# YOUNESELBOUKNIFY/CrossModal-IMU-Video-OOD-HAR

Measured on AMD Instinct MI355X. Metric: clips/sec fwd+bwd, 16x224^2 video + 200x6 IMU, batch 32, 1/2/4/8 GPU, higher is better.
Workload: dtype bf16; 1 GPU; CrossModalModel pretrain step: VideoMAE-B 16x224^2 + IMU 6x200 PatchTST, SigLIP loss, clip 1.0, AdamW; global_batch=32, per_gpu_batch=32, parallelism=dp1

## Files before the change

crossmodal-imu-video-ood-har_amd/cmhar/_lib.py:

```python
from __future__ import annotations

import ctypes as C
import os

import torch

_HERE = os.path.dirname(os.path.abspath(__file__))
LIB_PATH = os.environ.get('CMHAR_LIB', os.path.join(_HERE, 'libcmhar.so'))

F32, BF16, F16 = 0, 1, 2
ACT_NONE, ACT_GELU, ACT_RELU, ACT_DGELU, ACT_DRELU, ACT_GELU_SAVEGRAD, ACT_MULAUX = 0, 1, 2, 3, 4, 5, 6

vp, i32, i64, f32, u64 = C.c_void_p, C.c_int, C.c_long, C.c_float, C.c_ulonglong


class Epilogue(C.Structure):
    _fields_ = [('bias', vp), ('residual', vp), ('ldr', i64), ('aux_in', vp), ('lda', i64), ('aux_out', vp),
                ('ldo', i64), ('rowadd', vp), ('rowadd_mod', i32), ('rowadd_ld', i32), ('act', i32),
                ('alpha', f32), ('beta', f32), ('pdrop', f32), ('pad_', i32), ('seed', u64), ('rowsum', vp),
                ('rowsum_beta', f32), ('colscale_lo', i32), ('colscale_hi', i32), ('colscale', f32)]


class IMULayer(C.Structure):
    _fields_ = ([(n, vp) for n in ('w_qkv', 'b_qkv', 'w_out', 'b_out', 'ln1_g', 'ln1_b', 'w_ff1', 'b_ff1', 'w_ff2',
# ... 9 lines not shown
IMU_MAX_LAYERS = 8

_SIGS = {
    'cmhar_version': (i32, []),
    'cmhar_gemm_bf16': (i32, [i32, i32, i32, i32, i32, vp, i64, vp, i64, vp, i64, C.POINTER(Epilogue), i32, vp, vp]),
    'cmhar_gemm_bf16_phased': (i32, [i32, i32, i32, i32, i32, vp, i64, vp, i64, vp, i64, C.POINTER(Epilogue), i32, vp,
                                     vp, i32]),
    'cmhar_gemm_f16': (i32, [i32, i32, i32, i32, i32, vp, i64, vp, i64, vp, i64, C.POINTER(Epilogue), i32, vp, vp]),
    'cmhar_gemm_bf16_ws': (i64, [i32, i32, i32]),
    'cmhar_gemm_bf16_plan': (i32, [i32, i32, i32, i32, i32, i32, i32]),
    'cmhar_gemm_bf16_plan2': (i32, [i32, i32, i32, i32, i32, i32, i32, i32]),
    'cmhar_gemm_generic': (i32, [i32, i32, i32, i32, i32, i32, vp, i64, i64, i64, vp, i64, i64, i64, vp, i64, i64,
                                 C.POINTER(Epilogue), vp]),
    'cmhar_gemm_generic_splitk': (i32, [i32, i32, i32, i32, i32, i32, vp, i64, i64, vp, i64, i64, vp, i64,
                                        C.POINTER(Epilogue), vp, vp]),
    'cmhar_attention_fwd': (i32, [i32, i32, i32, i32, i32, i32, vp, i64, vp, i64, vp, i64, vp, i64, vp, f32, f32, u64,
                                  vp]),
    'cmhar_attention_fwd_opt': (i32, [i32]),
    'cmhar_attention_bwd': (i32, [i32, i32, i32, i32, i32, i32, vp, i64, vp, i64, vp, i64, vp, i64, vp, i64, vp, vp,
                                  vp, i64, vp, i64, vp, i64, f32, f32, u64, vp]),
    'cmhar_attention_bwd_prescaled': (i32, [i32, i32, i32, i32, vp, i64, vp, i64, vp, i64, vp, i64, vp, i64, vp, vp,
                                            vp, i64, vp, i64, vp, i64, f32, vp]),
    'cmhar_layernorm_fwd': (i32, [i32, i32, i32, vp, i64, vp, i64, f32, u64, vp, i64, vp, i64, vp, vp, vp, vp, f32,
                                  vp]),
    'cmhar_layernorm_bwd_ws': (i64, [i32, i32]),
    'cmhar_layernorm_bwd': (i32, [i32, i32, i32, vp, i64, vp, i64, vp, vp, vp, vp, i64, vp, i64, vp, i64, f32, u64,
                                  vp, vp, f32, vp, vp]),
    'cmhar_colsum_ws': (i64, [i32, i32]),
    'cmhar_colsum': (i32, [i32, i32, i32, vp, i64, vp, f32, f32, vp, i64, vp]),
    'cmhar_batchnorm_fwd': (i32, [i32, i32, vp, vp, vp, vp, vp, vp, vp, vp, i32, f32, f32, i32, vp, vp]),
    'cmhar_batchnorm_bwd': (i32, [i32, i32, vp, vp, vp, vp, vp, vp, vp, vp, vp, i32, i32, f32, vp]),
    'cmhar_l2normalize_fwd': (i32, [i32, i32, vp, vp, vp, f32, vp]),
    'cmhar_l2normalize_bwd': (i32, [i32, i32, vp, vp, vp, vp, f32, vp]),
    'cmhar_siglip_ws': (i64, [i32, i32]),
    'cmhar_siglip_loss': (i32, [i32, i32, i32, vp, vp, vp, vp, vp, vp, i32, i32, vp, i32, i32, vp, vp, vp, vp]),
    'cmhar_tubelet_im2col': (i32, [i32, i32, i32, i32, i32, i32, i32, i32, vp, vp, vp]),
    'cmhar_imu_embed_fwd': (i32, [i32, i32, i32, i32, i32, i32, i32, i32, vp, C.POINTER(vp), C.POINTER(vp), vp, vp,
                                  vp, vp]),
    'cmhar_imu_embed_bwd': (i32, [i32, i32, i32, i32, i32, i32, i32, i32, i32, vp, vp, vp, vp, C.POINTER(vp),
                                  C.POINTER(vp), vp]),
    'cmhar_imu_encoder_fwd': (i32, [i32, i32, i32, i32, i32, i32, vp, C.POINTER(IMULayer), vp, vp, f32, vp, vp, vp,
                                    f32, f32, u64, vp]),
    'cmhar_imu_encoder_bwd': (i32, [i32, i32, i32, i32, i32, i32, vp, C.POINTER(IMULayer), C.POINTER(IMULayerGrad),
                                    vp, vp, vp, vp, vp, vp, vp, f32, f32, u64, vp]),
    'cmhar_copy2d': (i32, [i32, i32, i32, i32, vp, i64, vp, i64, f32, f32, f32, u64, vp]),
    'cmhar_logits_energy': (i32, [i32, i32, i32, vp, i64, f32, vp, vp, vp, vp]),
    'cmhar_sim_topk_ws': (i64, [i32, i32, i32]),
    'cmhar_sim_topk_splits': (i32, [i32, i32, i32]),
    'cmhar_sim_topk': (i32, [i32, i32, i32, i32, i32, vp, i64, vp, i64, i64, vp, vp, vp, vp]),
    'cmhar_class_moments_ws': (i64, [i32, i32, i32]),
    'cmhar_class_moments': (i32, [i32, i32, i32, i32, vp, i64, vp, vp, vp, vp, vp, vp]),
    'cmhar_class_min_dist': (i32, [i32, i32, i32, i32, vp, i64, vp, i64, vp, i64, vp, vp, vp, i64, vp]),
    'cmhar_cross_entropy_ws': (i64, [i32]),
    'cmhar_resize_ksize': (i32, [i32, i32]),
    'cmhar_video_ingest_ws': (i64, [i32, i32, i32, i32, i32]),
    'cmhar_video_ingest': (i32, [i32, i32, vp, i64, i32, i32, vp, i32, i32, vp, vp, i32, vp, vp, i64, vp]),
    'cmhar_imu_preprocess_ws': (i64, [i64, i32, i32]),
    'cmhar_imu_preprocess': (i32, [i32, i32, vp, vp, i64, vp, i32, i32, i64, vp, vp, i32, vp, vp, vp]),
    'cmhar_cross_entropy': (i32, [i32, i32, vp, i64, i64, vp, i64, f32, f32, f32, i32, vp, vp, vp, vp, vp, vp, i64,
                                  i64, f32, f32, vp, vp, vp]),
    'cmhar_mt_grad_norm': (i32, [vp, vp, i32, vp, vp, f32, i32, vp]),
    'cmhar_mt_adamw': (i32, [vp, vp, i32, f32, f32, f32, f32, f32, f32, f32, vp, vp]),
    'cmhar_mt_adamw_clip': (i32, [vp, vp, i32, f32, f32, f32, f32, f32, f32, f32, vp, i32, vp]),
    'cmhar_mt_cast_bf16': (i32, [vp, vp, i32, vp]),
    'cmhar_conv3d_im2col': (i32, [i32, i32, vp, vp, vp, vp]),
    'cmhar_conv3d_col2im': (i32, [i32, vp, vp, vp, i32, vp]),
# ... 119 lines not shown
```

crossmodal-imu-video-ood-har_amd/cmhar/heads.py:

```python
from __future__ import annotations

import torch
import torch.nn as nn

from . import kernels as K
from ._lib import NoReplicate


def _blocks(seq: nn.Sequential):
    mods = list(seq)
    blocks, i = [], 0
    while i < len(mods) - 1:
        lin, bn, act = mods[i], mods[i + 1], mods[i + 2]
        if not (isinstance(lin, nn.Linear) and isinstance(bn, nn.BatchNorm1d) and isinstance(act, nn.ReLU)):
            raise TypeError('unsupported head structure')
        p, step = 0.0, 3
        if i + 3 < len(mods) and isinstance(mods[i + 3], nn.Dropout):
            p, step = mods[i + 3].p, 4
        blocks.append((lin, bn, p))
        i += step
    if not isinstance(mods[-1], nn.Linear):
        raise TypeError('head must end with a Linear')
    return blocks, mods[-1]

# ... 28 lines not shown
                                    bn_momentum(bn, upd), bn.eps, True,
                                    bn.num_batches_tracked if upd else None)
        pd = p if training else 0.0
        if pd > 0:
            yd = torch.empty_like(y)
            K.copy2d(y, yd, pdrop=pd, seed=seed + bi)
        else:
            yd = y
        if save:
            saved.append((h, z, y, sm, sr, pd, use_batch))
        h = yd
    out = K.linear(h, final.weight, final.bias)
    return out, (saved, h)


def _head_backward(seq, st, dout, seed):
    blocks, final = _blocks(seq)
    saved, hlast = st
    grads = {final.weight: K.linear_wgrad(dout, hlast), final.bias: K.colsum(dout)}
    dh = K.linear_dgrad(dout, final.weight)
    for bi in reversed(range(len(blocks))):
        lin, bn, _ = blocks[bi]
        h, z, y, sm, sr, pd, use_batch = saved[bi]
        if pd > 0:
            K.copy2d(dh, dh, pdrop=pd, seed=seed + bi)
        dz, dgw, dgb = K.batchnorm_bwd(z, y, dh, bn.weight, sm, sr, use_batch, True)
        grads[bn.weight], grads[bn.bias] = dgw, dgb
        grads[lin.weight] = K.linear_wgrad(dz, h)
        grads[lin.bias] = K.colsum(dz)
        dh = K.linear_dgrad(dz, lin.weight)
    return dh, grads


class _HeadFn(torch.autograd.Function):
    @staticmethod
    def forward(ctx, x, seq, training, seed, *params):
        out, st = _head_forward(seq, x, training, seed, save=True)
        ctx.seq, ctx.st, ctx.seed, ctx.params = seq, st, seed, params
        return out

    @staticmethod
    def backward(ctx, dout):
        dx, grads = _head_backward(ctx.seq, ctx.st, dout.contiguous(), ctx.seed)
        ctx.st = None
        return (dx, None, None, None) + tuple(grads.get(p) if p.requires_grad else None for p in ctx.params)


def run_head(seq: nn.Sequential, x: torch.Tensor, training: bool, seeds: _Seeds) -> torch.Tensor:
    if training and x.shape[0] <= 1:
        raise ValueError(f'Expected more than 1 value per channel when training, got input size {tuple(x.shape)}')
    x = x.contiguous().float()
    params = [p for p in seq.parameters()]
    has_drop = any(isinstance(m, nn.Dropout) and m.p > 0 for m in seq)
    seed = seeds.next() if (training and has_drop) else 0
    if torch.is_grad_enabled() and (x.requires_grad or any(p.requires_grad for p in params)):
        return _HeadFn.apply(x, seq, training, seed, *params)
    with torch.no_grad():
        return _head_forward(seq, x, training, seed, save=False)[0]


class ProjectionHead(NoReplicate, nn.Module):

    def __init__(self, in_dim, hidden_dim, out_dim):
        super().__init__()
        self.net = nn.Sequential(
            nn.Linear(in_dim, hidden_dim),
            nn.BatchNorm1d(hidden_dim),
            nn.ReLU(inplace=True),
            nn.Linear(hidden_dim, out_dim),
        )
        self._seeds = _Seeds()

    def forward(self, x):
        return run_head(self.net, x, self.training, self._seeds)


class _L2NormFn(torch.autograd.Function):
    @staticmethod
    def forward(ctx, x, eps):
        y, n = K.l2normalize_fwd(x, eps)
        ctx.save_for_backward(y, n)
        ctx.eps = eps
        return y

    @staticmethod
    def backward(ctx, dy):
        y, n = ctx.saved_tensors
        return K.l2normalize_bwd(y, dy, n, ctx.eps), None


def l2_normalize(x: torch.Tensor, eps: float = 1e-12) -> torch.Tensor:
    x = x.contiguous().float()
    if torch.is_grad_enabled() and x.requires_grad:
        return _L2NormFn.apply(x, eps)
    return K.l2normalize_fwd(x, eps)[0]
```

crossmodal-imu-video-ood-har_amd/cmhar/kernels.py:

```python
from __future__ import annotations

import ctypes as C
import math
import os

import torch

from . import _lib as L
from ._lib import call, ptr

class Tracer:
    def __init__(self):
        self.active = False
        self.only = None
        self.records = []

    def begin(self, name=None):
        if not self.active or (self.only is not None and name not in self.only):
            return None
        ev = torch.cuda.Event(enable_timing=True)
        ev.record()
        return ev

    def end(self, ev0, name, flops, nbytes):
# ... 416 lines not shown
    return y, sm, sr


def batchnorm_bwd(x, y, dy, w, sm, sr, training, relu, beta_acc=0.0, dw=None, db=None):
    B, Cc = x.shape
    dx = torch.empty_like(x)
    if dw is None:
        dw = torch.empty(Cc, dtype=torch.float32, device=x.device)
    if db is None:
        db = torch.empty(Cc, dtype=torch.float32, device=x.device)
    for t, n in ((dw, 'dw'), (db, 'db')):
        if t.dtype != torch.float32 or tuple(t.shape) != (Cc,) or not t.is_contiguous():
            raise ValueError(f'batchnorm_bwd: {n} must be a contiguous fp32 [{Cc}] tensor')
    call('cmhar_batchnorm_bwd', B, Cc, ptr(x), ptr(y), ptr(dy.contiguous()), ptr(w), ptr(sm), ptr(sr), ptr(dx),
         ptr(dw), ptr(db), int(training), int(relu), beta_acc, L.stream(x.device))
    return dx, dw, db


def l2normalize_fwd(x, eps=1e-12):
    M, N = x.shape
    y = torch.empty_like(x)
    nrm = torch.empty(M, dtype=torch.float32, device=x.device)
    call('cmhar_l2normalize_fwd', M, N, ptr(x), ptr(y), ptr(nrm), eps, L.stream(x.device))
    return y, nrm


def l2normalize_bwd(y, dy, nrm, eps=1e-12):
    M, N = y.shape
    dx = torch.empty_like(y)
    call('cmhar_l2normalize_bwd', M, N, ptr(y), ptr(dy.contiguous()), ptr(nrm), ptr(dx), eps, L.stream(y.device))
    return dx


def copy2d(src, dst, alpha=1.0, beta=0.0, pdrop=0.0, seed=0):
    _check_2d(src, 'src')
    _check_2d(dst, 'dst')
    if src.shape != dst.shape:
        raise ValueError('copy2d shape')
    call('cmhar_copy2d', L.dtype_code(src.dtype), L.dtype_code(dst.dtype), src.shape[0], src.shape[1], ptr(src),
         src.stride(0), ptr(dst), dst.stride(0), alpha, beta, pdrop, seed, L.stream(src.device))
    return dst


_REDUCTIONS = {'none': 0, 'mean': 1, 'sum': 2}


def cross_entropy(logits, labels=None, *, ignore_index=-100, label_smoothing=0.0, gamma=0.0, alpha=1.0,
                  reduction='mean', loss=None, row_loss=None, pred=None, correct=None, status=None, dlogits=None,
                  grad_scale=1.0, grad_beta=0.0, g_up=None):
    if logits.dim() != 2 or logits.dtype != torch.float32 or not logits.is_cuda:
        raise ValueError('logits: fp32 device matrix expected')
    N, Cc = logits.shape
    if labels is not None and (labels.dtype != torch.int64 or labels.shape != (N,) or not labels.is_contiguous()):
        raise ValueError(f'labels: contiguous int64 [{N}] expected')
    for t, n in ((row_loss, 'row_loss'), (pred, 'pred')):
        if t is not None and (t.numel() != N or not t.is_contiguous()):
            raise ValueError(f'{n}: [{N}] expected')
    if dlogits is not None and (tuple(dlogits.shape) != (N, Cc) or dlogits.dtype != torch.float32):
        raise ValueError('dlogits shape')
    red = _REDUCTIONS[reduction]
    if dlogits is not None and red == 0 and (g_up is None or g_up.numel() != N):
        raise ValueError("reduction='none' needs per-row upstream gradients")
    ws = workspace(L.lib().cmhar_cross_entropy_ws(N), logits.device)
    call('cmhar_cross_entropy', N, Cc, ptr(logits), logits.stride(0), logits.stride(1), ptr(labels), ignore_index,
         label_smoothing, gamma, alpha, red, ptr(loss), ptr(row_loss), ptr(pred), ptr(correct), ptr(status),
         ptr(dlogits), dlogits.stride(0) if dlogits is not None else 0,
# ... 21 lines not shown
```

crossmodal-imu-video-ood-har_amd/cmhar/models.py:

```python
from __future__ import annotations

import math
import os
import warnings

import torch
import torch.nn as nn

from . import kernels as K
from .heads import ProjectionHead, l2_normalize, run_head, _Seeds
from .imu import IMUEncoder, PatchEmbedding
from .cnn2d import MobileNetV2Features, ResNet18Features, run_cnn2d
from .fusion import _TokenMeanFn
from .r3d import R3D18, run_r3d
from .videomae import VideoMAEBackbone, default_videomae_config, run_backbone

__all__ = ['PatchEmbedding', 'IMUEncoder', 'VideoEncoder', 'ProjectionHead', 'CrossModalModel', 'IMUClassifier']


class _LinearFn(torch.autograd.Function):
    @staticmethod
    def forward(ctx, x, weight, bias):
        ctx.save_for_backward(x, weight)
        ctx.has_bias = bias is not None
        return K.linear(x, weight.detach(), None if bias is None else bias.detach())

    @staticmethod
    def backward(ctx, dy):
        x, w = ctx.saved_tensors
        dy = dy.contiguous()
        dx = K.linear_dgrad(dy, w.detach()) if ctx.needs_input_grad[0] else None
        dw = K.linear_wgrad(dy, x) if ctx.needs_input_grad[1] else None
        db = K.colsum(dy) if ctx.has_bias and ctx.needs_input_grad[2] else None
        return dx, dw, db


def linear_fp32(x, lin: nn.Linear):
    x = x.contiguous().float()
    if torch.is_grad_enabled() and (x.requires_grad or lin.weight.requires_grad):
        return _LinearFn.apply(x, lin.weight, lin.bias)
    return K.linear(x, lin.weight.detach(), None if lin.bias is None else lin.bias.detach())


def _videomae_geometry(config):
    m, d = config.model, config.data
    frames = m.videomae_num_frames or d.video_frames_per_window
    image = m.videomae_image_size or (d.video_resize[0] if isinstance(d.video_resize, (tuple, list)) else d.video_resize)
    return default_videomae_config(image_size=image, patch_size=m.videomae_patch_size, num_frames=frames,
                                   tubelet_size=m.videomae_tubelet_size, hidden_size=m.videomae_hidden_size,
                                   num_hidden_layers=m.videomae_num_layers, num_attention_heads=m.videomae_num_heads,
                                   intermediate_size=m.videomae_intermediate_size,
                                   layer_norm_eps=m.videomae_layer_norm_eps, qkv_bias=m.videomae_qkv_bias,
                                   use_mean_pooling=m.videomae_use_mean_pooling)


class VideoEncoder(nn.Module):

    def __init__(self, config):
        super().__init__()
        self.config = config
        model_cfg = config.model
        vb = model_cfg.video_backbone
        self.is_videomae = False
        dt = getattr(model_cfg, 'compute_dtype', 'bf16')
        if isinstance(vb, str) and ('videomae' in vb.lower() or '/' in vb):
            self.is_videomae = True
            if os.path.isdir(vb) and os.path.exists(os.path.join(vb, 'config.json')):
                self.backbone = VideoMAEBackbone.from_pretrained(vb, compute_dtype=dt)
            else:
                if model_cfg.video_pretrained:
                    allow = bool(getattr(model_cfg, 'allow_random_init', False)) or \
                        os.environ.get('CMHAR_ALLOW_RANDOM_INIT', '') == '1'
                    if not allow:
                        raise OSError(f'VideoMAE checkpoint {vb!r} cannot be loaded (not a local HF directory '
# ... 29 lines not shown

    def forward(self, x):
        if x.dim() != 5:
            raise ValueError(f'expected (B, T, C, H, W) video, got {tuple(x.shape)}')
        if isinstance(self.backbone, (ResNet18Features, MobileNetV2Features)):
            B, T = x.shape[:2]
            feats = linear_fp32(run_cnn2d(self.backbone, x, self.training), self.projection)
            return _TokenMeanFn.apply(feats, B, T)
        if not self.is_videomae:
            return linear_fp32(run_r3d(self.backbone, x, self.training), self.projection)
        feat = run_backbone(self.backbone, x, token0_only=True)
        return linear_fp32(feat, self.projection)


class CrossModalModel(nn.Module):

    def __init__(self, config):
        super().__init__()
        self.config = config
        model_cfg = config.model
        self.imu_encoder = IMUEncoder(config)
        self.video_encoder = VideoEncoder(config)
        self.imu_proj = ProjectionHead(model_cfg.imu_d_model, model_cfg.projection_hidden_dim,
                                       model_cfg.projection_dim)
        self.video_proj = ProjectionHead(model_cfg.video_d_model, model_cfg.projection_hidden_dim,
                                         model_cfg.projection_dim)
        self.temperature = nn.Parameter(torch.ones([]) * math.log(10))
        self.bias = nn.Parameter(torch.ones([]) * -10)
        self.overlap_imu = True
        self._side = {}

    def _imu_branch(self, imu):
        imu_feat, _ = self.imu_encoder(imu)
        return l2_normalize(self.imu_proj(imu_feat))

    def forward(self, imu, video):
        if self.overlap_imu and imu.is_cuda:
            cur = torch.cuda.current_stream(imu.device)
            side = self._side.get(imu.device)
            if side is None:
                side = self._side[imu.device] = torch.cuda.Stream(
                    imu.device, priority=int(os.environ.get('CMHAR_IMU_STREAM_PRIORITY', '0')))
            side.wait_stream(cur)
            with torch.cuda.stream(side):
                imu_out = self._imu_branch(imu)
            video_out = l2_normalize(self.video_proj(self.video_encoder(video)))
            cur.wait_stream(side)
            imu_out.record_stream(cur)
            return imu_out, video_out
        imu_out = self._imu_branch(imu)
        return imu_out, l2_normalize(self.video_proj(self.video_encoder(video)))


class IMUClassifier(nn.Module):

    def __init__(self, imu_encoder, config, freeze_encoder=False):
        super().__init__()
        self.imu_encoder = imu_encoder
        self.config = config
        model_cfg = config.model
        if freeze_encoder:
            for param in self.imu_encoder.parameters():
                param.requires_grad = False
        layers = []
        in_dim = model_cfg.imu_d_model
        for hidden_dim in model_cfg.classifier_hidden_dims:
            layers.extend([nn.Linear(in_dim, hidden_dim), nn.BatchNorm1d(hidden_dim), nn.ReLU(inplace=True),
                           nn.Dropout(model_cfg.classifier_dropout)])
            in_dim = hidden_dim
        layers.append(nn.Linear(in_dim, model_cfg.num_classes))
        self.classifier = nn.Sequential(*layers)
        self._seeds = _Seeds()

    def forward(self, imu):
        with torch.set_grad_enabled(self.training or not self.freeze_encoder):
            imu_feat, _ = self.imu_encoder(imu)
        return run_head(self.classifier, imu_feat, self.training, self._seeds)

    @property
    def freeze_encoder(self):
        return not next(self.imu_encoder.parameters()).requires_grad

    def unfreeze_encoder(self):
        for param in self.imu_encoder.parameters():
# ... 2 lines not shown
```

include/cmhar.h:

```cpp
#ifndef CMHAR_H
#define CMHAR_H
#include <hip/hip_runtime_api.h>

#ifdef __cplusplus
extern "C" {
#endif

typedef struct CmharEpilogue {
  const float* bias;
  const void* residual;
  long ldr;
  const void* aux_in;
  long lda;
  void* aux_out;
  long ldo;
  const float* rowadd;
  int rowadd_mod;
  int rowadd_ld;
  int act;
  float alpha;
  float beta;
  float pdrop;
  int pad_;
  unsigned long long seed;
// ... 30 lines not shown
int cmhar_attention_fwd_opt(int mode);
int cmhar_attention_bwd(int dtype, int B, int H, int Lq, int Lk, int D, const void* Q, long ldq, const void* K,
                        long ldk, const void* V, long ldv, const void* O, long ldo, const void* dO, long lddo,
                        const float* lse, float* delta, void* dQ, long lddq, void* dK, long lddk, void* dV, long lddv,
                        float scale, float pdrop, unsigned long long seed, hipStream_t stream);
int cmhar_attention_bwd_prescaled(int B, int H, int Lq, int Lk, const void* Q, long ldq, const void* K, long ldk,
                                  const void* V, long ldv, const void* O, long ldo, const void* dO, long lddo,
                                  const float* lse, float* delta, void* dQ, long lddq, void* dK, long lddk, void* dV,
                                  long lddv, float scale, hipStream_t stream);

int cmhar_layernorm_fwd(int dtype, int M, int N, const void* a, long lda, const void* b, long ldb, float pdrop,
                        unsigned long long seed, void* h_out, long ldh, void* y, long ldy, const float* gamma,
                        const float* beta, float* mean, float* rstd, float eps, hipStream_t stream);
long cmhar_layernorm_bwd_ws(int M, int N);
int cmhar_layernorm_bwd(int dtype, int M, int N, const void* dy, long lddy, const void* h, long ldh,
                        const float* gamma, const float* mean, const float* rstd, const void* dres, long ldres,
                        void* dh, long lddh, void* db_out, long lddb, float pdrop, unsigned long long seed,
                        float* dgamma, float* dbeta, float beta_acc, float* ws, hipStream_t stream);

long cmhar_colsum_ws(int M, int N);
int cmhar_colsum(int dtype, int M, int N, const void* X, long ldx, float* out, float alpha, float beta, float* ws,
                 long ws_floats, hipStream_t stream);

int cmhar_batchnorm_fwd(int B, int C, const float* x, float* y, const float* w, const float* bias, float* rmean,
                        float* rvar, float* smean, float* srstd, int training, float momentum, float eps, int relu,
                        long long* num_batches_tracked, hipStream_t stream);
int cmhar_batchnorm_bwd(int B, int C, const float* x, const float* y, const float* dy, const float* w,
                        const float* smean, const float* srstd, float* dx, float* dw, float* db, int training,
                        int relu, float beta_acc, hipStream_t stream);

int cmhar_l2normalize_fwd(int M, int N, const float* x, float* y, float* norm, float eps, hipStream_t stream);
int cmhar_l2normalize_bwd(int M, int N, const float* y, const float* dy, const float* norm, float* dx, float eps,
                          hipStream_t stream);

long cmhar_siglip_ws(int Ba, int Bb);
int cmhar_siglip_loss(int Ba, int Bb, int D, const float* a, const float* b, const float* t, const float* bias,
                      float* loss, float* da, int a_off, int a_cnt, float* db, int b_off, int b_cnt, float* gt,
                      float* gbias, float* ws, hipStream_t stream);

int cmhar_tubelet_im2col(int out_dtype, int B, int T, int C, int H, int W, int tub, int P, const float* video,
                         void* out, hipStream_t stream);

int cmhar_imu_embed_fwd(int B, int C, int L, int N, int P, int S, int D, int T, const float* x,
                        const float* const* w, const float* const* bias, const float* cls, const float* pos,
                        float* out, hipStream_t stream);
int cmhar_imu_embed_bwd(int B, int C, int L, int N, int P, int S, int D, int T, int Tpos, const float* x,
                        const float* dout, float* dcls, float* dpos, float* const* dw, float* const* db,
                        hipStream_t stream);

#define CMHAR_IMU_MAX_LAYERS 8
typedef struct CmharIMULayer {
  const float *w_qkv, *b_qkv, *w_out, *b_out, *ln1_g, *ln1_b, *w_ff1, *b_ff1, *w_ff2, *b_ff2, *ln2_g, *ln2_b;
  float eps1, eps2;
  float *qkv, *o, *lse, *s1, *mu1, *rs1, *h1, *fd, *s2, *mu2, *rs2, *h2;
} CmharIMULayer;
int cmhar_imu_encoder_fwd(int B, int T, int D, int H, int FF, int nlayers, const float* x, const CmharIMULayer* layers,
                          const float* norm_g, const float* norm_b, float norm_eps, float* enc, float* norm_mu,
                          float* norm_rs, float scale, float pdrop, unsigned long long seed, hipStream_t stream);
typedef struct CmharIMULayerGrad {
  float *dqkv, *da, *dpre, *df2, *gln1, *gln2;
  float *dw_qkv, *db_qkv, *dw_out, *db_out, *dln1_g, *dln1_b, *dw_ff1, *db_ff1, *dw_ff2, *db_ff2, *dln2_g, *dln2_b;
} CmharIMULayerGrad;
int cmhar_imu_encoder_bwd(int B, int T, int D, int H, int FF, int nlayers, const float* x, const CmharIMULayer* layers,
                          const CmharIMULayerGrad* grads, const float* norm_g, const float* norm_mu,
                          const float* norm_rs, const float* d_enc, float* dnorm_g, float* dnorm_b, float* dx,
                          float scale, float pdrop, unsigned long long seed, hipStream_t stream);
// ... 119 lines not shown
```

Before: 741.8 clips/sec.

## Add fused skinny-batch linear+BatchNorm+ReLU kernels for projection heads

Adds dedicated HIP kernels for small-batch (≤64 rows) fp32 linear layers. The forward kernel fuses bias, BatchNorm (batch or running stats, including running-stat updates) and ReLU into the GEMM. The backward kernel computes dx, dW, db and the BatchNorm or L2-normalize backward in one launch. Projection heads and generic small linears use these kernels, replacing separate linear, batchnorm, colsum and l2normalize launches, to cut launch count and tile waste at batch 32. The cost is a large amount of hand-written MFMA code whose correctness and numerics must match the unfused path.

```diff
diff --git a/crossmodal-imu-video-ood-har_amd/cmhar/_lib.py b/crossmodal-imu-video-ood-har_amd/cmhar/_lib.py
--- a/crossmodal-imu-video-ood-har_amd/cmhar/_lib.py
+++ b/crossmodal-imu-video-ood-har_amd/cmhar/_lib.py
@@ -65,6 +65,9 @@
     'cmhar_batchnorm_bwd': (i32, [i32, i32, vp, vp, vp, vp, vp, vp, vp, vp, vp, i32, i32, f32, vp]),
     'cmhar_l2normalize_fwd': (i32, [i32, i32, vp, vp, vp, f32, vp]),
     'cmhar_l2normalize_bwd': (i32, [i32, i32, vp, vp, vp, vp, f32, vp]),
+    'cmhar_skinny_linear_fwd': (i32, [i32, i32, i32, vp, vp, vp, vp, i32, vp, vp, vp, vp, vp, vp, vp, f32, f32, vp, vp]),
+    'cmhar_skinny_linear_bwd': (i32, [i32, i32, i32, vp, vp, vp, vp, vp, vp, i32, vp, vp, f32, vp, vp, vp, vp, vp, vp,
+                                      i32, vp]),
     'cmhar_siglip_ws': (i64, [i32, i32]),
     'cmhar_siglip_loss': (i32, [i32, i32, i32, vp, vp, vp, vp, vp, vp, i32, i32, vp, i32, i32, vp, vp, vp, vp]),
     'cmhar_tubelet_im2col': (i32, [i32, i32, i32, i32, i32, i32, i32, i32, vp, vp, vp]),
diff --git a/crossmodal-imu-video-ood-har_amd/cmhar/heads.py b/crossmodal-imu-video-ood-har_amd/cmhar/heads.py
--- a/crossmodal-imu-video-ood-har_amd/cmhar/heads.py
+++ b/crossmodal-imu-video-ood-har_amd/cmhar/heads.py
@@ -84,6 +84,64 @@
     return dh, grads
 
 
+def fused_ok(seq, x) -> bool:
+    blocks, final = _blocks(seq)
+    if x.dim() != 2 or any(p > 0 for _, _, p in blocks):
+        return False
+    if any(bn.weight is None or bn.bias is None or not K._f32c(bn.weight) or not K._f32c(bn.bias)
+           for _, bn, _ in blocks):
+        return False
+    lins = [b[0] for b in blocks] + [final]
+    if not K.skinny_ok(x, lins[0].weight, lins[0].bias):
+        return False
+    return all(lin.in_features % 4 == 0 and K._f32c(lin.weight) and lin.weight.data_ptr() % 16 == 0 and
+               (lin.bias is None or K._f32c(lin.bias)) for lin in lins[1:])
+
+
+def _bn_modes(bn, training):
+    upd = training and bn.track_running_stats and bn.running_mean is not None
+    use_batch = training or not bn.track_running_stats
+    return upd, use_batch
+
+
+def _head_forward_fused(seq, x, training, save, norm_eps=None):
+    blocks, final = _blocks(seq)
+    h = x
+    saved = []
+    for lin, bn, _ in blocks:
+        upd, use_batch = _bn_modes(bn, training)
+        stats = upd or not use_batch
+        y, z, sm, sr = K.skinny_linear_fwd(h, lin.weight, lin.bias, bn=dict(
+            weight=bn.weight, bias=bn.bias, rmean=bn.running_mean if stats else None,
+            rvar=bn.running_var if stats else None, batch_stats=use_batch, momentum=bn_momentum(bn, upd), eps=bn.eps,
+            num_batches_tracked=bn.num_batches_tracked if upd else None))
+        if save:
+            saved.append((h, z, y, sm, sr, use_batch))
+        h = y
+    out = K.skinny_linear_fwd(h, final.weight, final.bias)
+    nrm = None
+    if norm_eps is not None:
+        out, nrm = K.l2normalize_fwd(out, norm_eps)
+    return out, (saved, h, out if norm_eps is not None else None, nrm)
+
+
+def _head_backward_fused(seq, st, dout, need_dx, norm_eps=None):
+    blocks, final = _blocks(seq)
+    saved, hlast, yn, nrm = st
+    dh, dw, db = K.skinny_linear_bwd(dout, hlast, final.weight, need_dx=bool(blocks) or need_dx,
+                                     need_db=final.bias is not None,
+                                     l2n=(yn, nrm, norm_eps) if norm_eps is not None else None)
+    grads = {final.weight: dw, final.bias: db}
+    for bi in reversed(range(len(blocks))):
+        lin, bn, _ = blocks[bi]
+        h, z, y, sm, sr, use_batch = saved[bi]
+        dh, dw, db, dg, dbt = K.skinny_linear_bwd(dh, h, lin.weight, need_dx=bi > 0 or need_dx,
+                                                  need_db=lin.bias is not None,
+                                                  bn=(z, y, bn.weight, sm, sr, use_batch))
+        grads[bn.weight], grads[bn.bias], grads[lin.weight], grads[lin.bias] = dg, dbt, dw, db
+    return dh, grads
+
+
 class _HeadFn(torch.autograd.Function):
     @staticmethod
     def forward(ctx, x, seq, training, seed, *params):
@@ -98,11 +156,33 @@
         return (dx, None, None, None) + tuple(grads.get(p) if p.requires_grad else None for p in ctx.params)
 
 
-def run_head(seq: nn.Sequential, x: torch.Tensor, training: bool, seeds: _Seeds) -> torch.Tensor:
+class _FusedHeadFn(torch.autograd.Function):
+
+    @staticmethod
+    def forward(ctx, x, seq, training, norm_eps, *params):
+        out, st = _head_forward_fused(seq, x, training, True, norm_eps)
+        ctx.seq, ctx.st, ctx.norm_eps, ctx.params = seq, st, norm_eps, params
+        return out
+
+    @staticmethod
+    def backward(ctx, dout):
+        dx, grads = _head_backward_fused(ctx.seq, ctx.st, dout.contiguous(), ctx.needs_input_grad[0], ctx.norm_eps)
+        ctx.st = None
+        return (dx, None, None, None) + tuple(grads.get(p) if p.requires_grad else None for p in ctx.params)
+
+
+def run_head(seq: nn.Sequential, x: torch.Tensor, training: bool, seeds: _Seeds, norm_eps=None) -> torch.Tensor:
     if training and x.shape[0] <= 1:
         raise ValueError(f'Expected more than 1 value per channel when training, got input size {tuple(x.shape)}')
     x = x.contiguous().float()
     params = [p for p in seq.parameters()]
+    if fused_ok(seq, x):
+        if torch.is_grad_enabled() and (x.requires_grad or any(p.requires_grad for p in params)):
+            return _FusedHeadFn.apply(x, seq, training, norm_eps, *params)
+        with torch.no_grad():
+            return _head_forward_fused(seq, x, training, False, norm_eps)[0]
+    if norm_eps is not None:
+        return l2_normalize(run_head(seq, x, training, seeds), norm_eps)
     has_drop = any(isinstance(m, nn.Dropout) and m.p > 0 for m in seq)
     seed = seeds.next() if (training and has_drop) else 0
     if torch.is_grad_enabled() and (x.requires_grad or any(p.requires_grad for p in params)):
@@ -126,6 +206,9 @@
     def forward(self, x):
         return run_head(self.net, x, self.training, self._seeds)
 
+    def forward_normalized(self, x, eps: float = 1e-12):
+        return run_head(self.net, x, self.training, self._seeds, norm_eps=eps)
+
 
 class _L2NormFn(torch.autograd.Function):
     @staticmethod
diff --git a/crossmodal-imu-video-ood-har_amd/cmhar/kernels.py b/crossmodal-imu-video-ood-har_amd/cmhar/kernels.py
--- a/crossmodal-imu-video-ood-har_amd/cmhar/kernels.py
+++ b/crossmodal-imu-video-ood-har_amd/cmhar/kernels.py
@@ -472,6 +472,87 @@
     return dx
 
 
+HEADS_FUSED = os.environ.get('CMHAR_HEADS_FUSED', '1') != '0'
+SKINNY_MAX_ROWS = 64
+
+
+def _f32c(t):
+    return t.is_cuda and t.dtype == torch.float32 and t.is_contiguous()
+
+
+def skinny_ok(x, w, bias=None):
+    return (HEADS_FUSED and x.dim() == 2 and w.dim() == 2 and _f32c(x) and _f32c(w) and
+            (bias is None or _f32c(bias)) and 1 <= x.shape[0] <= SKINNY_MAX_ROWS and x.shape[1] == w.shape[1] and
+            x.shape[1] % 4 == 0 and x.data_ptr() % 16 == 0 and w.data_ptr() % 16 == 0)
+
+
+def _check_f32c(shape, **tensors):
+    for n, t in tensors.items():
+        if t is not None and (not _f32c(t) or (shape is not None and tuple(t.shape) != tuple(shape))):
+            raise ValueError(f'{n}: expected a contiguous fp32 device tensor' +
+                             (f' of shape {tuple(shape)}' if shape is not None else '') + f', got {tuple(t.shape)} '
+                             f'{t.dtype}')
+
+
+def skinny_linear_fwd(x, w, bias=None, *, bn=None):
+    B, K = x.shape
+    N = w.shape[0]
+    if not skinny_ok(x, w, bias):
+        raise ValueError(f'skinny_linear_fwd: unsupported operands x {tuple(x.shape)} w {tuple(w.shape)}')
+    _check_f32c((N,), bias=bias)
+    y = torch.empty(B, N, dtype=torch.float32, device=x.device)
+    if bn is None:
+        call('cmhar_skinny_linear_fwd', B, K, N, ptr(x), ptr(w), ptr(bias), ptr(y), 0, None, None, None, None, None,
+             None, None, 0.0, 0.0, None, L.stream(x.device))
+        return y
+    rmean, rvar, nbt = bn.get('rmean'), bn.get('rvar'), bn.get('num_batches_tracked')
+    _check_f32c((N,), bn_weight=bn['weight'], bn_bias=bn['bias'], rmean=rmean, rvar=rvar)
+    if nbt is not None and (nbt.dtype != torch.int64 or nbt.numel() != 1 or not nbt.is_cuda):
+        raise ValueError('num_batches_tracked: expected a device int64 scalar')
+    mode = 1 if bn['batch_stats'] else 2
+    if mode == 2 and (rmean is None or rvar is None):
+        raise ValueError('skinny_linear_fwd: running statistics needed without batch statistics')
+    z = torch.empty_like(y)
+    sm = torch.empty(N, dtype=torch.float32, device=x.device)
+    sr = torch.empty(N, dtype=torch.float32, device=x.device)
+    call('cmhar_skinny_linear_fwd', B, K, N, ptr(x), ptr(w), ptr(bias), ptr(y), mode, ptr(z), ptr(bn['weight']),
+         ptr(bn['bias']), ptr(rmean), ptr(rvar), ptr(sm), ptr(sr), float(bn['momentum']), float(bn['eps']),
+         ptr(nbt) if mode == 1 else None, L.stream(x.device))
+    return y, z, sm, sr
+
+
+def skinny_linear_bwd(dout, x, w, *, need_dx=True, need_db=True, l2n=None, bn=None):
+    B, K = x.shape
+    N = w.shape[0]
+    if not skinny_ok(x, w) or l2n is not None and bn is not None:
+        raise ValueError(f'skinny_linear_bwd: unsupported operands x {tuple(x.shape)} w {tuple(w.shape)}')
+    _check_f32c((B, N), dout=dout)
+    dev = x.device
+    dx = torch.empty(B, K, dtype=torch.float32, device=dev) if need_dx else None
+    dw = torch.empty(N, K, dtype=torch.float32, device=dev)
+    db = torch.empty(N, dtype=torch.float32, device=dev) if need_db else None
+    st = L.stream(dev)
+    if l2n is not None:
+        y, nrm, eps = l2n
+        _check_f32c((B, N), y=y)
+        _check_f32c((B,), norm=nrm)
+        call('cmhar_skinny_linear_bwd', B, K, N, ptr(dout), ptr(x), ptr(w), ptr(dx), ptr(dw), ptr(db), 1, ptr(y),
+             ptr(nrm), float(eps), None, None, None, None, None, None, 0, st)
+        return dx, dw, db
+    if bn is not None:
+        z, y, gw, sm, sr, batch_stats = bn
+        _check_f32c((B, N), z=z, y=y)
+        _check_f32c((N,), bn_weight=gw, smean=sm, srstd=sr)
+        dg = torch.empty(N, dtype=torch.float32, device=dev)
+        dbt = torch.empty(N, dtype=torch.float32, device=dev)
+        call('cmhar_skinny_linear_bwd', B, K, N, ptr(dout), ptr(x), ptr(w), ptr(dx), ptr(dw), ptr(db), 2, ptr(y),
+             None, 0.0, ptr(z), ptr(gw), ptr(sm), ptr(sr), ptr(dg), ptr(dbt), int(batch_stats), st)
+        return dx, dw, db, dg, dbt
+    call('cmhar_skinny_linear_bwd', B, K, N, ptr(dout), ptr(x), ptr(w), ptr(dx), ptr(dw), ptr(db), 0, None, None,
+         0.0, None, None, None, None, None, None, 0, st)
+    return dx, dw, db
+
+
 def copy2d(src, dst, alpha=1.0, beta=0.0, pdrop=0.0, seed=0):
     _check_2d(src, 'src')
     _check_2d(dst, 'dst')
diff --git a/crossmodal-imu-video-ood-har_amd/cmhar/models.py b/crossmodal-imu-video-ood-har_amd/cmhar/models.py
--- a/crossmodal-imu-video-ood-har_amd/cmhar/models.py
+++ b/crossmodal-imu-video-ood-har_amd/cmhar/models.py
@@ -8,7 +8,7 @@
 import torch.nn as nn
 
 from . import kernels as K
-from .heads import ProjectionHead, l2_normalize, run_head, _Seeds
+from .heads import ProjectionHead, run_head, _Seeds
 from .imu import IMUEncoder, PatchEmbedding
 from .cnn2d import MobileNetV2Features, ResNet18Features, run_cnn2d
 from .fusion import _TokenMeanFn
@@ -19,16 +19,24 @@
 
 
 class _LinearFn(torch.autograd.Function):
+
     @staticmethod
     def forward(ctx, x, weight, bias):
         ctx.save_for_backward(x, weight)
         ctx.has_bias = bias is not None
+        ctx.skinny = K.skinny_ok(x, weight, bias)
+        if ctx.skinny:
+            return K.skinny_linear_fwd(x, weight.detach(), None if bias is None else bias.detach())
         return K.linear(x, weight.detach(), None if bias is None else bias.detach())
 
     @staticmethod
     def backward(ctx, dy):
         x, w = ctx.saved_tensors
         dy = dy.contiguous()
+        if ctx.skinny and ctx.needs_input_grad[1]:
+            dx, dw, db = K.skinny_linear_bwd(dy, x, w.detach(), need_dx=ctx.needs_input_grad[0],
+                                             need_db=ctx.has_bias and ctx.needs_input_grad[2])
+            return dx, dw, db
         dx = K.linear_dgrad(dy, w.detach()) if ctx.needs_input_grad[0] else None
         dw = K.linear_wgrad(dy, x) if ctx.needs_input_grad[1] else None
         db = K.colsum(dy) if ctx.has_bias and ctx.needs_input_grad[2] else None
@@ -39,7 +47,8 @@
     x = x.contiguous().float()
     if torch.is_grad_enabled() and (x.requires_grad or lin.weight.requires_grad):
         return _LinearFn.apply(x, lin.weight, lin.bias)
-    return K.linear(x, lin.weight.detach(), None if lin.bias is None else lin.bias.detach())
+    w, b = lin.weight.detach(), None if lin.bias is None else lin.bias.detach()
+    return K.skinny_linear_fwd(x, w, b) if K.skinny_ok(x, w, b) else K.linear(x, w, b)
 
 
 def _videomae_geometry(config):
@@ -135,7 +144,7 @@
 
     def _imu_branch(self, imu):
         imu_feat, _ = self.imu_encoder(imu)
-        return l2_normalize(self.imu_proj(imu_feat))
+        return self.imu_proj.forward_normalized(imu_feat)
 
     def forward(self, imu, video):
         if self.overlap_imu and imu.is_cuda:
@@ -147,12 +156,12 @@
             side.wait_stream(cur)
             with torch.cuda.stream(side):
                 imu_out = self._imu_branch(imu)
-            video_out = l2_normalize(self.video_proj(self.video_encoder(video)))
+            video_out = self.video_proj.forward_normalized(self.video_encoder(video))
             cur.wait_stream(side)
             imu_out.record_stream(cur)
             return imu_out, video_out
         imu_out = self._imu_branch(imu)
-        return imu_out, l2_normalize(self.video_proj(self.video_encoder(video)))
+        return imu_out, self.video_proj.forward_normalized(self.video_encoder(video))
 
 
 class IMUClassifier(nn.Module):
diff --git a/crossmodal-imu-video-ood-har_amd/csrc/heads_fused.hip b/crossmodal-imu-video-ood-har_amd/csrc/heads_fused.hip
--- /dev/null
+++ b/crossmodal-imu-video-ood-har_amd/csrc/heads_fused.hip
@@ -0,0 +1,384 @@
+#include "rowops.h"
+
+namespace {
+
+constexpr int SK_NW = 8, SK_NT = SK_NW * 64;
+constexpr int SK_MAXB = 64;
+constexpr int SK_RLD = 17;
+constexpr int SK_DYF = 12544;
+
+__device__ __forceinline__ floatx4 ld4(const float* p, bool ok) {
+  if (ok) return *(const floatx4*)p;
+  return floatx4{0.f, 0.f, 0.f, 0.f};
+}
+__device__ __forceinline__ float ld1(const float* p, bool ok) { return ok ? *p : 0.f; }
+
+struct SkinnyBN {
+  int mode;
+  float* z;
+  const float* gamma;
+  const float* beta;
+  float* rmean;
+  float* rvar;
+  float* smean;
+  float* srstd;
+  float momentum, eps;
+  long long* nbt;
+};
+
+template <int NBT>
+__global__ __launch_bounds__(SK_NT) void skinny_fwd_kernel(int B, int K, int N, int nc, const float* __restrict__ x,
+                                                           const float* __restrict__ W,
+                                                           const float* __restrict__ bias, float* __restrict__ y,
+                                                           SkinnyBN bn) {
+  __shared__ float red[SK_NW][NBT * 16][SK_RLD];
+  __shared__ float stat[2][16];
+  const int tid = threadIdx.x, lane = tid & 63, w = tid >> 6;
+  const int r = lane & 15, g = lane >> 4;
+  const int n0 = blockIdx.x * nc;
+  const bool nok = r < nc && n0 + r < N;
+  const float* wp = W + (long)(nok ? n0 + r : 0) * K;
+  const float* xp[NBT];
+  bool bok[NBT];
+#pragma unroll
+  for (int bt = 0; bt < NBT; ++bt) {
+    bok[bt] = bt * 16 + r < B;
+    xp[bt] = x + (long)(bok[bt] ? bt * 16 + r : 0) * K;
+  }
+  const int je = tid & 15;
+  const bool jok = je < nc && n0 + je < N;
+  const float bj = ld1(bias + (jok ? n0 + je : 0), jok && bias);
+  const float gj = ld1(bn.gamma + (jok ? n0 + je : 0), jok && bn.mode);
+  const float bej = ld1(bn.beta + (jok ? n0 + je : 0), jok && bn.mode);
+  floatx4 acc[NBT];
+#pragma unroll
+  for (int bt = 0; bt < NBT; ++bt) acc[bt] = floatx4{0.f, 0.f, 0.f, 0.f};
+  constexpr int U = NBT <= 2 ? 3 : 2;
+  for (int kb = w * 32; kb < K; kb += U * SK_NW * 32) {
+    floatx4 wf[U][2], xf[U][NBT][2];
+#pragma unroll
+    for (int u = 0; u < U; ++u) {
+      const int k = kb + u * SK_NW * 32 + 8 * g;
+      const bool k0ok = k < K, k1ok = k + 4 < K;
+      wf[u][0] = ld4(wp + k, nok && k0ok);
+      wf[u][1] = ld4(wp + k + 4, nok && k1ok);
+#pragma unroll
+      for (int bt = 0; bt < NBT; ++bt) {
+        xf[u][bt][0] = ld4(xp[bt] + k, bok[bt] && k0ok);
+        xf[u][bt][1] = ld4(xp[bt] + k + 4, bok[bt] && k1ok);
+      }
+    }
+#pragma unroll
+    for (int u = 0; u < U; ++u)
+#pragma unroll
+      for (int h = 0; h < 2; ++h)
+#pragma unroll
+        for (int e = 0; e < 4; ++e)
+#pragma unroll
+          for (int bt = 0; bt < NBT; ++bt)
+            acc[bt] = __builtin_amdgcn_mfma_f32_16x16x4f32(xf[u][bt][h][e], wf[u][h][e], acc[bt], 0, 0, 0);
+  }
+#pragma unroll
+  for (int bt = 0; bt < NBT; ++bt)
+#pragma unroll
+    for (int rr = 0; rr < 4; ++rr) red[w][bt * 16 + 4 * g + rr][r] = acc[bt][rr];
+  __syncthreads();
+  for (int idx = tid; idx < NBT * 256; idx += SK_NT) {
+    const int b = idx >> 4, j = idx & 15, n = n0 + j;
+    float s = red[0][b][j];
+#pragma unroll
+    for (int ww = 1; ww < SK_NW; ++ww) s += red[ww][b][j];
+    const bool ok = b < B && j < nc && n < N;
+    if (ok && bias) s += bj;
+    red[0][b][j] = s;
+    if (ok) (bn.mode ? bn.z : y)[(long)b * N + n] = s;
+  }
+  if (!bn.mode) return;
+  __syncthreads();
+  if (tid < 16 && tid < nc && n0 + tid < N) {
+    const int c = n0 + tid;
+    float mu, rs;
+    if (bn.mode == 1) {
+      float s = 0.f;
+      for (int b = 0; b < B; ++b) s += red[0][b][tid];
+      mu = s / B;
+      float q = 0.f;
+      for (int b = 0; b < B; ++b) { const float d = red[0][b][tid] - mu; q += d * d; }
+      const float var = q / B;
+      rs = rsqrtf(var + bn.eps);
+      if (bn.rmean) {
+        bn.rmean[c] = (1.f - bn.momentum) * bn.rmean[c] + bn.momentum * mu;
+        bn.rvar[c] = (1.f - bn.momentum) * bn.rvar[c] + bn.momentum * var * B / (B - 1);
+      }
+    } else {
+      mu = bn.rmean[c];
+      rs = rsqrtf(bn.rvar[c] + bn.eps);
+    }
+    bn.smean[c] = mu;
+    bn.srstd[c] = rs;
+    stat[0][tid] = mu;
+    stat[1][tid] = rs;
+  }
+  if (blockIdx.x == 0 && tid == 0 && bn.mode == 1 && bn.nbt) *bn.nbt += 1;
+  __syncthreads();
+  for (int idx = tid; idx < NBT * 256; idx += SK_NT) {
+    const int b = idx >> 4, j = idx & 15, n = n0 + j;
+    if (b < B && j < nc && n < N) {
+      const float v = (red[0][b][j] - stat[0][j]) * stat[1][j] * gj + bej;
+      y[(long)b * N + n] = fmaxf(v, 0.f);
+    }
+  }
+}
+
+struct SkinnyPro {
+  int mode;
+  const float* y;
+  const float* norm;
+  float eps;
+  const float* z;
+  const float* gamma;
+  const float* smean;
+  const float* srstd;
+  float* dgamma;
+  float* dbeta;
+  int training;
+};
+
+template <int NBT>
+__global__ __launch_bounds__(SK_NT) void skinny_bwd_kernel(int B, int K, int N, int nch, const float* __restrict__ dout,
+                                                           const float* __restrict__ x, const float* __restrict__ W,
+                                                           float* __restrict__ dx, float* __restrict__ dW,
+                                                           float* __restrict__ db, SkinnyPro pro) {
+  __shared__ float smem[SK_DYF];
+  __shared__ float rowdot[SK_MAXB], rownorm[SK_MAXB];
+  const int tid = threadIdx.x, lane = tid & 63, w = tid >> 6;
+  const int r = lane & 15, g = lane >> 4;
+  const int k0 = blockIdx.x * 16;
+  const bool kok = k0 + r < K;
+  const int LD = nch + 2;
+  constexpr int B16 = NBT * 16;
+
+  float xr[NBT * 4];
+#pragma unroll
+  for (int s = 0; s < NBT * 4; ++s) {
+    const int b = 4 * s + g;
+    xr[s] = ld1(x + (long)(b < B ? b : 0) * K + (kok ? k0 + r : 0), kok && b < B);
+  }
+  if (pro.mode == 1) {
+    constexpr int RW = (B16 + SK_NW - 1) / SK_NW;
+    float s[RW];
+#pragma unroll
+    for (int i = 0; i < RW; ++i) s[i] = 0.f;
+    for (int c = lane; c < N; c += 256) {
+      float yv[4][RW], dv[4][RW];
+#pragma unroll
+      for (int u = 0; u < 4; ++u)
+#pragma unroll
+        for (int i = 0; i < RW; ++i) {
+          const bool ok = w + SK_NW * i < B && c + 64 * u < N;
+          const long o = ok ? (long)(w + SK_NW * i) * N + c + 64 * u : 0;
+          yv[u][i] = ld1(pro.y + o, ok);
+          dv[u][i] = ld1(dout + o, ok);
+        }
+#pragma unroll
+      for (int u = 0; u < 4; ++u)
+#pragma unroll
+        for (int i = 0; i < RW; ++i) s[i] += yv[u][i] * dv[u][i];
+    }
+#pragma unroll
+    for (int i = 0; i < RW; ++i) {
+      const int bb = w + SK_NW * i;
+      const float t = wave_sum(s[i]);
+      if (lane == 0 && bb < B) { rowdot[bb] = t; rownorm[bb] = pro.norm[bb]; }
+    }
+    __syncthreads();
+  }
+  floatx4 adx[NBT];
+#pragma unroll
+  for (int bt = 0; bt < NBT; ++bt) adx[bt] = floatx4{0.f, 0.f, 0.f, 0.f};
+
+  for (int c0 = 0; c0 < N; c0 += nch) {
+    constexpr int WU = 12;
+    float wf[WU];
+    if (dx) {
+#pragma unroll
+      for (int u = 0; u < WU; ++u) {
+        const int nn = 4 * w + 4 * SK_NW * u, n = c0 + nn + g;
+        const bool ok = kok && n < N && nn < nch;
+        wf[u] = ld1(W + (ok ? (long)n * K + k0 + r : 0), ok);
+      }
+    }
+    if (pro.mode == 2) {
+      constexpr int RB = 32;
+      for (int nn = tid; nn < nch; nn += SK_NT) {
+        const int c = c0 + nn;
+        if (c < N) {
+          const float mu = pro.smean[c], rs = pro.srstd[c], wr = pro.gamma[c] * rs;
+          float gq[RB], xh[RB];
+          auto rows = [&](int b0) {
+#pragma unroll
+            for (int i = 0; i < RB; ++i) {
+              const bool ok = b0 + i < B;
+              const int o = (ok ? b0 + i : 0) * N + c;
+              const float d = dout[o], ya = pro.y[o], zz = pro.z[o];
+              gq[i] = ok && ya > 0.f ? d : 0.f;
+              xh[i] = (zz - mu) * rs;
+            }
+          };
+          float sg = 0.f, sgx = 0.f;
+          for (int b0 = 0; b0 < B; b0 += RB) {
+            rows(b0);
+#pragma unroll
+            for (int i = 0; i < RB; ++i) { sg += gq[i]; sgx += gq[i] * xh[i]; }
+          }
+          if (blockIdx.x == 0) { pro.dgamma[c] = sgx; pro.dbeta[c] = sg; }
+          const float mg = pro.training ? sg / B : 0.f, mgx = pro.training ? sgx / B : 0.f;
+          for (int b0 = 0; b0 < B16; b0 += RB) {
+            if (B > RB) rows(b0);
+#pragma unroll
+            for (int i = 0; i < RB; ++i)
+              if (b0 + i < B16) smem[(b0 + i) * LD + nn] = b0 + i < B ? wr * (gq[i] - mg - xh[i] * mgx) : 0.f;
+          }
+        } else {
+          for (int b = 0; b < B16; ++b) smem[b * LD + nn] = 0.f;
+        }
+      }
+    } else {
+      constexpr int RPT = B16 / 4;
+      const int tc = tid & 127, rg = tid >> 7;
+      for (int nn = tc; nn < nch; nn += 128) {
+        const int c = c0 + nn;
+        float v[RPT], yv[RPT];
+#pragma unroll
+        for (int i = 0; i < RPT; ++i) {
+          const int bb = rg + 4 * i;
+          const bool ok = bb < B && c < N;
+          const int o = ok ? bb * N + c : 0;
+          const float d = dout[o];
+          v[i] = ok ? d : 0.f;
+          yv[i] = pro.mode == 1 ? pro.y[o] : 0.f;
+        }
+#pragma unroll
+        for (int i = 0; i < RPT; ++i) {
+          const int bb = rg + 4 * i;
+          float t = v[i];
+          if (pro.mode == 1 && bb < B) {
+            const float nr = rownorm[bb];
+            t = nr > pro.eps ? (t - yv[i] * rowdot[bb]) / nr : t / pro.eps;
+          }
+          smem[bb * LD + nn] = t;
+        }
+      }
+    }
+    __syncthreads();
+    if (db && blockIdx.x == 0) {
+      for (int nn = tid; nn < nch; nn += SK_NT) {
+        if (c0 + nn < N) {
+          float s = 0.f;
+          for (int b = 0; b < B; ++b) s += smem[b * LD + nn];
+          db[c0 + nn] = s;
+        }
+      }
+    }
+    if (dx) {
+#pragma unroll
+      for (int u = 0; u < WU; ++u) {
+        if (4 * w + 4 * SK_NW * u < nch) {
+#pragma unroll
+          for (int bt = 0; bt < NBT; ++bt)
+            adx[bt] = __builtin_amdgcn_mfma_f32_16x16x4f32(smem[(bt * 16 + r) * LD + 4 * w + 4 * SK_NW * u + g], wf[u],
+                                                           adx[bt], 0, 0, 0);
+        }
+      }
+      for (int nn = 4 * w + 4 * SK_NW * WU; nn < nch; nn += 4 * SK_NW) {
+        const int n = c0 + nn + g;
+        const bool ok = kok && n < N;
+        const float wl = ld1(W + (ok ? (long)n * K + k0 + r : 0), ok);
+#pragma unroll
+        for (int bt = 0; bt < NBT; ++bt)
+          adx[bt] = __builtin_amdgcn_mfma_f32_16x16x4f32(smem[(bt * 16 + r) * LD + nn + g], wl, adx[bt], 0, 0, 0);
+      }
+    }
+    for (int nt = w; nt * 16 < nch && c0 + nt * 16 < N; nt += SK_NW) {
+      floatx4 a = floatx4{0.f, 0.f, 0.f, 0.f};
+#pragma unroll
+      for (int s = 0; s < NBT * 4; ++s)
+        a = __builtin_amdgcn_mfma_f32_16x16x4f32(smem[(4 * s + g) * LD + nt * 16 + r], xr[s], a, 0, 0, 0);
+#pragma unroll
+      for (int rr = 0; rr < 4; ++rr) {
+        const int n = c0 + nt * 16 + 4 * g + rr;
+        if (n < N && kok) dW[(long)n * K + k0 + r] = a[rr];
+      }
+    }
+    __syncthreads();
+  }
+  if (!dx) return;
+  float* red = smem;
+#pragma unroll
+  for (int bt = 0; bt < NBT; ++bt)
+#pragma unroll
+    for (int rr = 0; rr < 4; ++rr) red[(w * B16 + bt * 16 + 4 * g + rr) * SK_RLD + r] = adx[bt][rr];
+  __syncthreads();
+  for (int idx = tid; idx < B16 * 16; idx += SK_NT) {
+    const int b = idx >> 4, j = idx & 15;
+    float s = red[b * SK_RLD + j];
+#pragma unroll
+    for (int ww = 1; ww < SK_NW; ++ww) s += red[(ww * B16 + b) * SK_RLD + j];
+    if (b < B && k0 + j < K) dx[(long)b * K + k0 + j] = s;
+  }
+}
+
+static_assert(SK_NW * SK_MAXB * SK_RLD <= SK_DYF, "dx partial tiles must fit the dy image");
+
+inline bool aligned16(const void* p) { return ((uintptr_t)p & 15) == 0; }
+
+}
+
+extern "C" int cmhar_skinny_linear_fwd(int B, int K, int N, const float* x, const float* W, const float* bias,
+                                       float* y, int bn_mode, float* z, const float* gamma, const float* beta,
+                                       float* rmean, float* rvar, float* smean, float* srstd, float momentum,
+                                       float eps, long long* num_batches_tracked, hipStream_t st) {
+  if (B <= 0 || N <= 0) return 0;
+  if (B > SK_MAXB || K <= 0 || K % 4 || !aligned16(x) || !aligned16(W) || !x || !W || !y) return -1;
+  if (bn_mode < 0 || bn_mode > 2) return -1;
+  if (bn_mode && (!z || !gamma || !beta || !smean || !srstd)) return -1;
+  if (bn_mode == 2 && (!rmean || !rvar)) return -1;
+  if (bn_mode == 1 && (!rmean) != (!rvar)) return -1;
+  SkinnyBN bn{bn_mode, z, gamma, beta, rmean, rvar, smean, srstd, momentum, eps, num_batches_tracked};
+  const int nc = cdiv(N, 16) >= 32 ? 16 : 8;
+  const int grid = cdiv(N, nc);
+  switch (cdiv(B, 16)) {
+    case 1: skinny_fwd_kernel<1><<<grid, SK_NT, 0, st>>>(B, K, N, nc, x, W, bias, y, bn); break;
+    case 2: skinny_fwd_kernel<2><<<grid, SK_NT, 0, st>>>(B, K, N, nc, x, W, bias, y, bn); break;
+    case 3: skinny_fwd_kernel<3><<<grid, SK_NT, 0, st>>>(B, K, N, nc, x, W, bias, y, bn); break;
+    default: skinny_fwd_kernel<4><<<grid, SK_NT, 0, st>>>(B, K, N, nc, x, W, bias, y, bn); break;
+  }
+  CMHAR_CHECK_LAUNCH();
+  return 0;
+}
+
+extern "C" int cmhar_skinny_linear_bwd(int B, int K, int N, const float* dout, const float* x, const float* W,
+                                       float* dx, float* dW, float* db, int pro_mode, const float* py,
+                                       const float* norm, float eps, const float* z, const float* gamma,
+                                       const float* smean, const float* srstd, float* dgamma, float* dbeta,
+                                       int training, hipStream_t st) {
+  if (B <= 0 || N <= 0 || K <= 0) return 0;
+  if (B > SK_MAXB || !dout || !x || !W || !dW) return -1;
+  if (pro_mode < 0 || pro_mode > 2) return -1;
+  if (pro_mode == 1 && (!py || !norm)) return -1;
+  if (pro_mode == 2 && (!py || !z || !gamma || !smean || !srstd || !dgamma || !dbeta)) return -1;
+  SkinnyPro pro{pro_mode, py, norm, eps, z, gamma, smean, srstd, dgamma, dbeta, training};
+  const int nbt = cdiv(B, 16);
+  int nch = ((SK_DYF / (nbt * 16) - 2) / 64) * 64;
+  const int n64 = cdiv(N, 64) * 64;
+  if (nch > n64) nch = n64;
+  const int grid = cdiv(K, 16);
+  switch (nbt) {
+    case 1: skinny_bwd_kernel<1><<<grid, SK_NT, 0, st>>>(B, K, N, nch, dout, x, W, dx, dW, db, pro); break;
+    case 2: skinny_bwd_kernel<2><<<grid, SK_NT, 0, st>>>(B, K, N, nch, dout, x, W, dx, dW, db, pro); break;
+    case 3: skinny_bwd_kernel<3><<<grid, SK_NT, 0, st>>>(B, K, N, nch, dout, x, W, dx, dW, db, pro); break;
+    default: skinny_bwd_kernel<4><<<grid, SK_NT, 0, st>>>(B, K, N, nch, dout, x, W, dx, dW, db, pro); break;
+  }
+  CMHAR_CHECK_LAUNCH();
+  return 0;
+}
diff --git a/include/cmhar.h b/include/cmhar.h
--- a/include/cmhar.h
+++ b/include/cmhar.h
@@ -86,6 +86,15 @@
 int cmhar_l2normalize_fwd(int M, int N, const float* x, float* y, float* norm, float eps, hipStream_t stream);
 int cmhar_l2normalize_bwd(int M, int N, const float* y, const float* dy, const float* norm, float* dx, float eps,
                           hipStream_t stream);
+
+int cmhar_skinny_linear_fwd(int B, int K, int N, const float* x, const float* W, const float* bias, float* y,
+                            int bn_mode, float* z, const float* gamma, const float* beta, float* rmean, float* rvar,
+                            float* smean, float* srstd, float momentum, float eps, long long* num_batches_tracked,
+                            hipStream_t stream);
+int cmhar_skinny_linear_bwd(int B, int K, int N, const float* dout, const float* x, const float* W, float* dx,
+                            float* dW, float* db, int pro_mode, const float* y, const float* norm, float eps,
+                            const float* z, const float* gamma, const float* smean, const float* srstd,
+                            float* dgamma, float* dbeta, int training, hipStream_t stream);
 
 long cmhar_siglip_ws(int Ba, int Bb);
 int cmhar_siglip_loss(int Ba, int Bb, int D, const float* a, const float* b, const float* t, const float* bias,
```

Measured after the change: 746.3 clips/sec, median of 6. About the same (+0.6%).
